# amazon-science/siam-mot

Measured on AMD Instinct MI355X. Metric: frame-pairs/sec at 720p, 30 active tracks; EMM xcorr HBM GB/s vs peak, higher is better.
Workload: dtype f32 (towers and correlation: fp16x2 operands on MFMA, fp32 accumulate, fp32-equivalent error); 1 GPU; EMM tracker-head frame pair (EMM.forward + EMM.extract_cache) on DLA-34-FPN 720p FPN maps (net input 704x1280, C=128, 5 levels), 30 tracks, one stream per GPU; hot path only: backbone / RPN / box head / solver are outside the timed region; tracks=30, channels=128, rz=15, rx=30, feature_sets=8, feature_bytes_rotated=307281920

## Files before the change

siam-mot_amd/csrc/sr_xcorr.hip:

```cpp
#include "pool_launch.h"
#include "xcorr_patch2.h"
#include "xcorr_patch1.h"
#include "xcorr_f16x2.h"
#include "knobs.h"
#include <type_traits>

namespace smot {

constexpr int FX_CH = 8;

struct SrOut {
    float* sr;
    float pad, half_e, two_e, min_wh;
    long long* trace;
    int abl;
    const int* n_valid;
    int order;
    float* hint_out;
    const float* hint_in;
    int hint_extra;
    int plan_pad[SMOT_MAX_LEVELS];
    float* plane_max;
};
constexpr int HINT_FLOATS = SMOT_HINT_FLOATS;
constexpr int HINT_BOUNDS = 8, HINT_GEOM = 12, HINT_YTAB = 16, HINT_XTAB = 16 + 256;
constexpr int HINT_BYROI = HINT_XTAB + 256, HINT_STATUS = HINT_BYROI + 6;
static_assert(HINT_BYROI + 8 == HINT_FLOATS && (HINT_FLOATS * 4) % 32 == 0 && HINT_STATUS == SMOT_HINT_STATUS_WORD,
              "hint entry layout");

typedef const __attribute__((address_space(1))) char* gptr_t;
__device__ __forceinline__ float ld_off(gptr_t base, unsigned byte_off) {
    return *reinterpret_cast<const __attribute__((address_space(1))) float*>(base + byte_off);
}
__device__ __forceinline__ gptr_t uniform_base(const float* p) {
    unsigned long long a = reinterpret_cast<unsigned long long>(p);
    asm volatile("" : "+s"(a));
    return reinterpret_cast<gptr_t>(a);
}

#ifdef SMOT_DEBUG
#include "../../measure/csrc/sr_xcorr_gen2.inc"
#endif

typedef int v4i_t __attribute__((ext_vector_type(4)));

typedef int v2i_t __attribute__((ext_vector_type(2)));
template <typename FT>
struct fx_pair {
    typedef int type;
};
template <>
struct fx_pair<float> {
    typedef v2i_t type;
};
template <typename FT>
__device__ __forceinline__ typename fx_pair<FT>::type fx_load2(__amdgpu_buffer_rsrc_t rsrc, unsigned voff, int soff) {
    if constexpr (sizeof(FT) == 4) {
        return __builtin_amdgcn_raw_buffer_load_b64(rsrc, voff, soff, 0);
    } else {
        return __builtin_amdgcn_raw_buffer_load_b32(rsrc, voff, soff, 0);
    }
}
template <typename FT>
__device__ __forceinline__ float fx_pair_elem(typename fx_pair<FT>::type v, int k) {
    if constexpr (sizeof(FT) == 4) {
        return __int_as_float(v[k]);
    } else {
        return k == 0 ? feat_of_pair<FT, 0>((unsigned)v) : feat_of_pair<FT, 1>((unsigned)v);
    }
}
template <typename FT>
__device__ __forceinline__ float fx_load1(__amdgpu_buffer_rsrc_t rsrc, unsigned voff, int soff) {
    if constexpr (sizeof(FT) == 4) {
        return __int_as_float(__builtin_amdgcn_raw_buffer_load_b32(rsrc, voff, soff, 0));
    } else {
        return feat_cvt<FT>((unsigned short)__builtin_amdgcn_raw_buffer_load_b16(rsrc, voff, soff, 0));
    }
}

__device__ __forceinline__ float rl_f(float v, int lane_const) {
    return __int_as_float(__builtin_amdgcn_readlane(__float_as_int(v), lane_const));
}

__device__ __forceinline__ float4 search_region_of(float b0, float b1, float b2, float b3, const SrOut& S) {
    const float bx1 = add_rn(b0, S.pad), by1 = add_rn(b1, S.pad);
    const float bx2 = add_rn(b2, S.pad), by2 = add_rn(b3, S.pad);
    const float bw = add_rn(sub_rn(bx2, bx1), 1.0f), bh = add_rn(sub_rn(by2, by1), 1.0f);
    const float w_ext = max_nan(div_rn(sub_rn(S.min_wh, bw), S.two_e), mul_rn(bw, S.half_e));
    const float h_ext = max_nan(div_rn(sub_rn(S.min_wh, bh), S.two_e), mul_rn(bh, S.half_e));
    return make_float4(sub_rn(bx1, w_ext), sub_rn(by1, h_ext), add_rn(bx2, w_ext), add_rn(by2, h_ext));
}

template <int RXN, int G>
__device__ __forceinline__ void fx_write_hint(const LevelParams& P, const float* __restrict__ boxes, const SrOut& S,
                                              const int* n_valid, float* hint_out, int NT, int x, int wave, int lane) {
    if (NT > 256 || wave >= 2) return;
    const int nv = (n_valid != nullptr) ? min(*n_valid + S.hint_extra, NT) : NT;
    if (x >= nv) return;
    unsigned long long mask[4][3];
    int cnt[3] = {0, 0, 0};
    int cl[4];
#pragma unroll
    for (int p = 0; p < 4; ++p) {
        const int t = lane + 64 * p;
        cl[p] = -1;
        if (64 * p < nv && t < nv) {
            const float4 b4 = *reinterpret_cast<const float4*>(boxes + (size_t)t * 4);
            int lvl = 0;
            if (P.num_levels > 1) lvl = map_level(boxes + (size_t)t * 4, P.k_min, P.k_max);
            float scale = P.scale[0];
#pragma unroll
            for (int l = 1; l < SMOT_MAX_LEVELS; ++l) scale = (lvl == l) ? P.scale[l] : scale;
            const float4 srb = search_region_of(b4.x, b4.y, b4.z, b4.w, S);
            const float ww = (srb.z - srb.x) * scale;
            cl[p] = ww <= 30.0f ? 0 : (ww <= 62.0f ? 1 : 2);
        }
#pragma unroll
        for (int c = 0; c < 3; ++c) {
            mask[p][c] = __ballot(cl[p] == c);
            cnt[c] += __popcll(mask[p][c]);
        }
    }
    const int px = x >> 6, lx = x & 63;
    int cx = 0;
#pragma unroll
    for (int p = 0; p < 4; ++p)
        if (p == px) cx = __builtin_amdgcn_readlane(cl[p], lx);
    int rank = cx == 2 ? 0 : (cx == 1 ? cnt[2] : cnt[2] + cnt[1]);
#pragma unroll
    for (int p = 0; p < 4; ++p) {
        const unsigned long long mk = cx == 2 ? mask[p][2] : (cx == 1 ? mask[p][1] : mask[p][0]);
        if (p < px) rank += __popcll(mk);
        if (p == px) rank += __popcll(mk & ((1ull << lx) - 1ull));
    }
    const float* bx = boxes + (size_t)x * 4;
    const float4 roi = search_region_of(bx[0], bx[1], bx[2], bx[3], S);
    int lvl = 0;
    if (P.num_levels > 1) lvl = map_level(bx, P.k_min, P.k_max);
    lvl = __builtin_amdgcn_readfirstlane(lvl);
    const int H = P.H[lvl], W = P.W[lvl], pad = S.plan_pad[lvl];
    const float scale = P.scale[lvl];
    const float x1 = mul_rn(roi.x, scale), y1 = mul_rn(roi.y, scale);
    const float x2 = mul_rn(roi.z, scale), y2 = mul_rn(roi.w, scale);
    const float bin_h = div_rn(fmaxf(sub_rn(y2, y1), 1.0f), (float)RXN);
    const float bin_w = div_rn(fmaxf(sub_rn(x2, x1), 1.0f), (float)RXN);
    int* ent = reinterpret_cast<int*>(hint_out) + (size_t)rank * HINT_FLOATS;
    int lo = 0, hi = 0;
    float wl = 0.0f, wh = 0.0f;
    if (lane < RXN * G) {
        if (wave == 0) {
            axis_sample(y1, bin_h, G, lane, H, pad, &lo, &hi, &wl, &wh);
        } else {
            axis_sample(x1, bin_w, G, lane, W, pad, &lo, &hi, &wl, &wh);
        }
    }
    int mn = 0x7fffffff, mx = -1;
    const unsigned long long m = __ballot(wl != 0.0f || wh != 0.0f);
    if (m != 0ull) {
        mn = __builtin_amdgcn_readlane((wl != 0.0f) ? lo : hi, __ffsll((long long)m) - 1);
        mx = __builtin_amdgcn_readlane((wh != 0.0f) ? hi : lo, 63 - __clzll((long long)m));
    }
    const int rl = (wl != 0.0f) ? lo : mn, rh = (wh != 0.0f) ? hi : mn;
    int4 e;
    if (wave == 0) {
        e.x = (int)((unsigned)(rl * W) * 4u);
        e.y = (int)((unsigned)(rh * W) * 4u);
    } else {
        e.x = (wl != 0.0f) ? lo - mn : 0;
        e.y = (wh != 0.0f) ? hi - mn : 0;
    }
    e.z = __float_as_int(wl);
    e.w = __float_as_int(wh);
    *reinterpret_cast<int4*>(ent + (wave == 0 ? HINT_YTAB : HINT_XTAB) + 4 * lane) = e;
    if (lane == 0) {
        ent[HINT_BOUNDS + 2 * wave] = mn;
        ent[HINT_BOUNDS + 2 * wave + 1] = mx;
        if (wave == 0) {
            float4* o = reinterpret_cast<float4*>(ent);
            o[0] = roi;
            o[1] = make_float4(__int_as_float(lvl), __int_as_float(x), 0.f, 0.f);
            ent[HINT_GEOM + 0] = pad;
            ent[HINT_GEOM + 1] = H;
            ent[HINT_GEOM + 2] = W;
            ent[HINT_GEOM + 3] = __float_as_int(scale);
            int* rec = reinterpret_cast<int*>(hint_out) + (size_t)x * HINT_FLOATS + HINT_BYROI;
            float4* r4 = reinterpret_cast<float4*>(rec);
            r4[0] = roi;
            rec[4] = lvl;
            rec[5] = nv;
            rec[6] = 0;
            rec[7] = 0;
        }
    }
}

__device__ __forceinline__ void fx_verify_hint(const LevelParams& P, const float* __restrict__ sr,
                                               const float* __restrict__ boxes, const float* hint, int x, int NT, int lane) {
    const int* rec = reinterpret_cast<const int*>(hint) + (size_t)x * HINT_FLOATS + HINT_BYROI;
    int v = 0;
    if (lane < 4) {
        v = __float_as_int(sr[(size_t)x * 4 + lane]);
    } else if (lane < 8) {
        v = __float_as_int(boxes[(size_t)x * 4 + lane - 4]);
    } else if (lane < 14) {
        v = rec[lane - 8];
    }
    const int up = __shfl_up(v, 8);
    float b4[4];
#pragma unroll
    for (int i = 0; i < 4; ++i) b4[i] = __int_as_float(__builtin_amdgcn_readlane(v, 4 + i));
    int lvl = 0;
    if (P.num_levels > 1) lvl = map_level(b4, P.k_min, P.k_max);
    const bool bad = (lane >= 8 && lane < 12 && up != v) || (lane == 12 && v != lvl) || (lane == 13 && v != NT);
    if (__ballot(bad) != 0ull && lane == 0)
        atomicOr(reinterpret_cast<int*>(const_cast<float*>(hint)) + HINT_STATUS, 1);
}

__device__ __forceinline__ bool fx_assign(const LevelParams& P, const float* __restrict__ sr,
                                          const float* __restrict__ boxes, const int* __restrict__ n_valid, int order,
                                          int by, int ny, const float* __restrict__ hint, int NT, int lane, int* n_out,
                                          int* cg_out, float4* roi_out, int* lvl_out, int* k_out) {
    int n = blockIdx.x, cg = by;
    *n_out = n;
    *cg_out = cg;
    if (order == 0 || NT > 256 || NT < 2) return false;
    const int T = NT * ny, L = by * NT + blockIdx.x;
    if (hint != nullptr && order == 1 && n_valid == nullptr) {
        const int k = L / ny;
        *cg_out = L - k * ny;
        *k_out = k;
        typedef int v8i_t __attribute__((ext_vector_type(8)));
        const v8i_t e = *reinterpret_cast<const __attribute__((address_space(4))) v8i_t*>(
            reinterpret_cast<unsigned long long>(hint) + (unsigned long long)k * (HINT_FLOATS * 4));
        roi_out->x = __int_as_float(e[0]);
        roi_out->y = __int_as_float(e[1]);
        roi_out->z = __int_as_float(e[2]);
        roi_out->w = __int_as_float(e[3]);
        *lvl_out = min(max(e[4], 0), P.num_levels - 1);
        *n_out = min(max(e[5], 0), NT - 1);
        return true;
    }
    const int nv = (n_valid != nullptr) ? min(*n_valid, NT) : NT;
    constexpr int SLOTS = 256;
    int i = L;
    if (order == 2) {
        const int r = L / SLOTS, q = L - r * SLOTS;
        if (r == 1) {
            i = T - 1 - q;
        } else if (r >= 2) {
            i = SLOTS + (L - 2 * SLOTS);
        }
    }
    int k;
    if (order == 3) {
        k = blockIdx.x;
    } else {
        k = i / ny;
        cg = i - k * ny;
    }
    *cg_out = cg;
    if (k >= nv) {
        *n_out = k;
        return false;
    }
    unsigned long long mask[4][3];
    int cnt[3] = {0, 0, 0};
    float rbx[4], rby[4], rbz[4], rbw[4];
    int rl[4];
#pragma unroll
    for (int p = 0; p < 4; ++p) {
        int cls = -1;
        const int t = lane + 64 * p;
        rbx[p] = rby[p] = rbz[p] = rbw[p] = 0.0f;
        rl[p] = 0;
        if (64 * p < nv && t < nv) {
            int lvl = 0;
            if (P.num_levels > 1) lvl = map_level(boxes + (size_t)t * 4, P.k_min, P.k_max);
            float scale = P.scale[0];
#pragma unroll
            for (int l = 1; l < SMOT_MAX_LEVELS; ++l) scale = (lvl == l) ? P.scale[l] : scale;
            const float4 b4 = *reinterpret_cast<const float4*>(sr + (size_t)t * 4);
            rbx[p] = b4.x;
            rby[p] = b4.y;
            rbz[p] = b4.z;
            rbw[p] = b4.w;
            rl[p] = lvl;
            const float ww = (b4.z - b4.x) * scale;
            cls = ww <= 30.0f ? 0 : (ww <= 62.0f ? 1 : 2);
        }
#pragma unroll
        for (int c = 0; c < 3; ++c) {
            mask[p][c] = __ballot(cls == c);
            cnt[c] += __popcll(mask[p][c]);
        }
    }
    int m = k, csel = 2;
    if (m >= cnt[2]) {
        m -= cnt[2];
        csel = 1;
        if (m >= cnt[1]) {
            m -= cnt[1];
            csel = 0;
        }
    }
    int psel = 0;
    bool done = false;
    unsigned long long msel = 0ull;
#pragma unroll
    for (int p = 0; p < 4; ++p) {
        const unsigned long long mk = csel == 2 ? mask[p][2] : (csel == 1 ? mask[p][1] : mask[p][0]);
        const int pc = __popcll(mk);
        if (!done) {
            if (m < pc) {
                psel = p;
                msel = mk;
                done = true;
            } else {
                m -= pc;
            }
        }
    }
    const unsigned long long below = msel & ((1ull << lane) - 1ull);
    const bool hit = ((msel >> lane) & 1ull) != 0ull && __popcll(below) == m;
    const unsigned long long b = __ballot(hit);
    if (b == 0ull) return false;
    const int ln = __ffsll((long long)b) - 1;
    *n_out = ln + 64 * psel;
    float sx = rbx[0], sy = rby[0], sz = rbz[0], sw = rbw[0];
    int lsel = rl[0];
#pragma unroll
    for (int p = 1; p < 4; ++p)
        if (psel == p) {
            sx = rbx[p];
            sy = rby[p];
            sz = rbz[p];
            sw = rbw[p];
            lsel = rl[p];
        }
    roi_out->x = __int_as_float(__builtin_amdgcn_readlane(__float_as_int(sx), ln));
    roi_out->y = __int_as_float(__builtin_amdgcn_readlane(__float_as_int(sy), ln));
    roi_out->z = __int_as_float(__builtin_amdgcn_readlane(__float_as_int(sz), ln));
    roi_out->w = __int_as_float(__builtin_amdgcn_readlane(__float_as_int(sw), ln));
    *lvl_out = __builtin_amdgcn_readlane(lsel, ln);
    return true;
}


#define FX_LEAD_PARAMS                                                                                                  \
    float *hint, const int *n_valid, const float *__restrict__ sr, const float *__restrict__ boxes,                     \
        long long *__restrict__ trace, int order, int grid_nx, int grid_ny, int C
#define FX_TAIL_PARAMS                                                                                                  \
    const float *__restrict__ z, float *__restrict__ resp, float *__restrict__ x_debug, int32_t *__restrict__ levels_out, \
        LevelParams P, SrOut S
template <int RX, int RZ, int G, bool XCORR, int NCH = FX_CH, bool P2 = false, int MM = 0>
__global__ void __launch_bounds__(64 * NCH, (P2 || MM == 1) ? 4 : 6)
sr_xcorr_fused9_kernel(FX_LEAD_PARAMS, FX_TAIL_PARAMS) {
    constexpr bool BATCHED = false;
    constexpr NoImages I{};
    using FT = float;
    constexpr bool NHWC = false;
#include "sr_xcorr_fused9_body.h"
}

template <int RX, int RZ, int G, bool XCORR, int NCH = FX_CH, int MM = 0>
__global__ void __launch_bounds__(64 * NCH, MM == 1 ? 4 : 6)
sr_xcorr_fused9_batched_kernel(FX_LEAD_PARAMS, FX_TAIL_PARAMS, ImageRows I) {
    constexpr bool BATCHED = true;
    constexpr bool P2 = false;
    using FT = float;
    constexpr bool NHWC = false;
#include "sr_xcorr_fused9_body.h"
}

template <typename FT, int RX, int RZ, int G, bool XCORR, int MM = 0>
__global__ void __launch_bounds__(64 * FX_CH, MM == 1 ? 4 : 6)
sr_xcorr_fused9_half_kernel(FX_LEAD_PARAMS, FX_TAIL_PARAMS) {
    static_assert(sizeof(FT) == 2, "fp16 / bf16 maps");
    constexpr bool BATCHED = false;
    constexpr NoImages I{};
    constexpr int NCH = FX_CH;
    constexpr bool P2 = false;
    constexpr bool NHWC = false;
#include "sr_xcorr_fused9_body.h"
}
// ... 246 lines not shown
```

siam-mot_amd/csrc/sr_xcorr_fused9_body.h:

```cpp
    constexpr int HO = XCORR ? RX - RZ + 1 : 16;
    constexpr int NS = RX * G;
    constexpr int XS = P2 ? XP2_XS : (MM == 2 ? XL_XS : XP1_XS), XP = P2 ? XP2_XP : (MM == 2 ? 30 * XL_XS : 32 * XP1_XS), ZS = XP1_ZS,
                  ZP = MM == 1 ? XH_TZ_FLOATS : (MM == 2 ? XL_TZ_FLOATS : RZ * XP1_ZS);
    static_assert(MM == 0 || (XCORR && !P2 && RX == 30 && RZ == 15), "the matrix-pipe correlation is the 30 / 15 head's");
    static_assert(MM != 2 || ((XP * 4) % 128 == 0 && ((2 * XP + 2 * ZP) * 4) % 128 == 0), "lean layout: 128-byte aligned plane images");
    constexpr int RH = (RX + 1) / 2;
    static_assert((!XCORR || RX - RZ + 1 == 16) && RX <= 32 && G == 2 && RX * XS <= XP && 2 * RH * G <= 64,
                  "specialised for pooled sizes <= 32, g = 2 (and the 30/15/16 correlation geometry)");
    __shared__ __attribute__((aligned(128))) float sm[(NCH / 2) * (2 * XP + 2 * ZP)];
    __shared__ __attribute__((aligned(16))) int4 tab[2][64 + 2 * RH * G];
    __shared__ int wbound[4];

    const int tid = threadIdx.x;
    const int lane = tid & 63;
    const int wave = __builtin_amdgcn_readfirstlane(tid >> 6);
    const float* const hint_in = XCORR ? hint : nullptr;
    float* const hint_out = XCORR ? nullptr : hint;
    const long long t_start = trace ? (long long)__builtin_amdgcn_s_memtime() : 0ll;
    float roi_early[4] = {0.0f, 0.0f, 0.0f, 0.0f};
    if constexpr (RX <= 15) {
#pragma unroll
        for (int k = 0; k < 4; ++k) roi_early[k] = sr[(size_t)blockIdx.x * 4 + k];
    }
    const int ka_h = P.H[0], ka_w = P.W[0], ka_p = P.pad[0];
    const float ka_s = P.scale[0];
    const unsigned long long ka_f = reinterpret_cast<unsigned long long>(P.feat[0]);
#define SMOT_KA_USE() asm volatile("" ::"s"(ka_h), "s"(ka_w), "s"(ka_p), "s"(ka_s), "s"(ka_f))
    int ka_i[6] = {0, 0, 0, 0, 0, 0};
    if constexpr (BATCHED) {
        ka_i[0] = I.num_images;
#pragma unroll
        for (int k = 1; k < 6; ++k) ka_i[k] = I.row_start[min(16 * k - 1, SMOT_MAX_IMAGES)];
    }
#ifdef SMOT_DEBUG
    if (S.abl >= 100 && (int)(blockIdx.y * grid_nx + blockIdx.x) >= 256) {
        for (int d = 0; d < S.abl - 100; ++d) __builtin_amdgcn_s_sleep(8);
    }
#endif
    int n_assigned, cg_assigned, lvl_assigned = 0;
    float4 roi_assigned = make_float4(0.f, 0.f, 0.f, 0.f);
    int grid_row = blockIdx.y, grid_rows = grid_ny;
    if constexpr (!XCORR) {
        if (hint_out != nullptr) {
            if (grid_row == 0) {
                fx_write_hint<30, G>(P, boxes, S, n_valid, hint_out, grid_nx, blockIdx.x, wave, lane);
                return;
            }
            grid_row -= 1;
            grid_rows -= 1;
        }
    }
    int4 tab_early = make_int4(0, 0, 0, 0);
    int4 ye_early = make_int4(0, 0, 0, 0), xe_early[2] = {make_int4(0, 0, 0, 0), make_int4(0, 0, 0, 0)};
    typedef int v8h_t __attribute__((ext_vector_type(8)));
    v8h_t g8 = {0, 0, 0, 0, -1, -1, -1, 0};
    if constexpr (XCORR && RX == 30) {
        if (hint_in != nullptr && order == 1 && n_valid == nullptr && grid_nx >= 2 && grid_nx <= 256) {
            const int k0 = (int)(blockIdx.y * grid_nx + blockIdx.x) / grid_ny;
            const int* ent = reinterpret_cast<const int*>(hint_in) + (size_t)k0 * HINT_FLOATS;
            g8 = *reinterpret_cast<const __attribute__((address_space(4))) v8h_t*>(
                reinterpret_cast<unsigned long long>(ent) + 4ull * HINT_BOUNDS);
            if (wave < 2) tab_early = *reinterpret_cast<const int4*>(ent + (wave == 0 ? HINT_YTAB : HINT_XTAB) + 4 * lane);
            if constexpr (MM == 1) {
                ye_early = *reinterpret_cast<const int4*>(ent + HINT_YTAB + 4 * min(lane + (wave & 1) * RH * G, 63));
                const int pwl = (lane & 31) < RX ? (lane & 31) : 0;
                xe_early[0] = *reinterpret_cast<const int4*>(ent + HINT_XTAB + 4 * (pwl * G));
                xe_early[1] = *reinterpret_cast<const int4*>(ent + HINT_XTAB + 4 * (pwl * G + 1));
            }
        }
    }
    if constexpr (XCORR && RX == 30) {
        if (hint_in != nullptr && order == 1 && n_valid == nullptr && grid_nx >= 2 && grid_nx <= 256 &&
            blockIdx.y == 0 && wave == 2
#ifdef SMOT_DEBUG
            && S.abl != 6
#endif
        )
            fx_verify_hint(P, sr, boxes, hint_in, blockIdx.x, grid_nx, lane);
    }
    int k_assigned = -1;
    const bool have_roi = fx_assign(P, sr, boxes, n_valid, RX > 15 ? order : 0, grid_row, grid_rows,
                                    XCORR ? hint_in : nullptr, grid_nx, lane, &n_assigned, &cg_assigned, &roi_assigned,
                                    &lvl_assigned, &k_assigned);
    SMOT_KA_USE();
#undef SMOT_KA_USE
    if constexpr (BATCHED)
        asm volatile("" ::"s"(ka_i[0]), "s"(ka_i[1]), "s"(ka_i[2]), "s"(ka_i[3]), "s"(ka_i[4]), "s"(ka_i[5]));
    const int n = __builtin_amdgcn_readfirstlane(n_assigned);
    const int cgrp = __builtin_amdgcn_readfirstlane(cg_assigned);
    if (n_valid != nullptr && n >= *n_valid) return;
    int img = 0;
    if constexpr (BATCHED) img = image_of_row(I, n);
#define FX_TRACE(SLOT)                                                                      \
    if (trace && tid == 0)                                                                  \
        trace[((size_t)n * grid_rows + cgrp) * 8 + (SLOT)] = (long long)__builtin_amdgcn_s_memtime();
    if (trace && tid == 0) trace[((size_t)n * grid_rows + cgrp) * 8 + 0] = t_start;
    FX_TRACE(5)

    float roi0 = roi_assigned.x, roi1 = roi_assigned.y, roi2 = roi_assigned.z, roi3 = roi_assigned.w;
    int lvl = lvl_assigned;
    if (!have_roi) {
        if constexpr (RX <= 15) {
            roi0 = roi_early[0];
            roi1 = roi_early[1];
            roi2 = roi_early[2];
            roi3 = roi_early[3];
        } else {
            roi0 = sr[(size_t)n * 4 + 0];
            roi1 = sr[(size_t)n * 4 + 1];
            roi2 = sr[(size_t)n * 4 + 2];
            roi3 = sr[(size_t)n * 4 + 3];
        }
        lvl = 0;
        if (P.num_levels > 1) lvl = map_level(boxes + (size_t)n * 4, P.k_min, P.k_max);
    }
    const float roi[4] = {roi0, roi1, roi2, roi3};
    lvl = __builtin_amdgcn_readfirstlane(lvl);
    if (levels_out != nullptr && cgrp == 0 && tid == 0) levels_out[n] = lvl;
    if (!XCORR && S.sr != nullptr && cgrp == 0 && tid == 0) {
        const float4 o = search_region_of(roi[0], roi[1], roi[2], roi[3], S);
        S.sr[n * 4 + 0] = o.x;
        S.sr[n * 4 + 1] = o.y;
        S.sr[n * 4 + 2] = o.z;
        S.sr[n * 4 + 3] = o.w;
    }
    const int H = P.H[lvl], W = P.W[lvl], pad = P.pad[lvl];
    const float scale = P.scale[lvl];
    const float x1 = mul_rn(roi[0], scale), y1 = mul_rn(roi[1], scale);
    const float x2 = mul_rn(roi[2], scale), y2 = mul_rn(roi[3], scale);
    const float bin_h = div_rn(fmaxf(sub_rn(y2, y1), 1.0f), (float)RX);
    const float bin_w = div_rn(fmaxf(sub_rn(x2, x1), 1.0f), (float)RX);
    FX_TRACE(6)
    constexpr int nplanes = NCH;
    const int c0 = cgrp * NCH;
    const bool owns = (wave < nplanes && c0 + wave < C);
    const int plane = n * C + c0 + wave;
    constexpr int NZ = XCORR ? (RZ * RZ + 63) / 64 : 1;
    float zreg[NZ];
    float zq[4] = {0.0f, 0.0f, 0.0f, 0.0f}, isz = 1.0f;
    if constexpr (MM != 0) {
        if (owns) xh_template_load(z + (size_t)plane * (RZ * RZ), lane, zq);
    } else if (XCORR && owns) {
        const float* __restrict__ zg = z + (size_t)plane * (RZ * RZ);
#pragma unroll
        for (int t = 0; t < NZ; ++t) zreg[t] = zg[min(lane + 64 * t, RZ * RZ - 1)];
    }

    const bool hent = XCORR && RX == 30 && k_assigned >= 0 && g8[4] == pad && g8[5] == H && g8[6] == W &&
                      g8[7] == __float_as_int(scale);
    const int hb[4] = {g8[0], g8[1], g8[2], g8[3]};
    const bool fast = !NHWC && MM == 1 && hent && hb[3] - hb[2] + 1 <= 64
#ifdef SMOT_DEBUG
                      && S.abl != 3 && S.abl != 12
#endif
        ;
    if (fast) {
    } else if (wave < 2 && hent) {
        tab[wave][lane] = tab_early;
        if (lane < 2 * RH * G) tab[wave][64 + lane] = make_int4(0, 0, 0, 0);
    } else if (wave < 2) {
        int lo = 0, hi = 0;
        float wl = 0.0f, wh = 0.0f;
        if (lane < NS) {
            if (wave == 0) {
                axis_sample(y1, bin_h, G, lane, H, pad, &lo, &hi, &wl, &wh);
            } else {
                axis_sample(x1, bin_w, G, lane, W, pad, &lo, &hi, &wl, &wh);
            }
        }
        int mn = 0x7fffffff, mx = -1;
        const unsigned long long m = __ballot(wl != 0.0f || wh != 0.0f);
        if (m != 0ull) {
            mn = __builtin_amdgcn_readlane((wl != 0.0f) ? lo : hi, __ffsll((long long)m) - 1);
            mx = __builtin_amdgcn_readlane((wh != 0.0f) ? hi : lo, 63 - __clzll((long long)m));
        }
        const int rl = (wl != 0.0f) ? lo : mn, rh = (wh != 0.0f) ? hi : mn;
        int4 e;
        if (wave == 0) {
            e.x = (int)((unsigned)(rl * W) * 4u);
            e.y = (int)((unsigned)(rh * W) * 4u);
        } else {
            e.x = (wl != 0.0f) ? lo - mn : 0;
            e.y = (wh != 0.0f) ? hi - mn : 0;
        }
        e.z = __float_as_int(wl);
        e.w = __float_as_int(wh);
        tab[wave][lane] = e;
        if (lane < 2 * RH * G) tab[wave][64 + lane] = make_int4(0, 0, 0, 0);
        if (lane == 0) {
            wbound[2 * wave] = mn;
            wbound[2 * wave + 1] = mx;
        }
    }
    FX_TRACE(7)
    if (!fast) __syncthreads();
    const int ymin = hent ? hb[0] : wbound[0], ymax = hent ? hb[1] : wbound[1];
    const int xmin = hent ? hb[2] : wbound[2], xmax = hent ? hb[3] : wbound[3];
    if (ymax < ymin || xmax < xmin) {
        if (owns) {
            if (XCORR) {
                for (int e = lane; e < HO * HO; e += 64) resp[(size_t)plane * HO * HO + e] = 0.0f;
                if (S.plane_max != nullptr && lane == 0) S.plane_max[plane] = 0.0f;
            }
            if (x_debug != nullptr)
                for (int e = lane; e < RX * RX; e += 64) x_debug[(size_t)plane * RX * RX + e] = 0.0f;
        }
        return;
    }
    const int ww = xmax - xmin + 1;
    FX_TRACE(1)

    if constexpr (MM != 0) {
    } else if (XCORR && owns) {
        float* zs = sm + (wave >> 1) * (2 * XP + 2 * ZP) + 2 * XP + (wave & 1) * ZP;
#pragma unroll
        for (int t = 0; t < NZ; ++t) {
            const int e = lane + 64 * t;
            if (e < RZ * RZ) {
                const int u = e / RZ;
                zs[u * ZS + (e - u * RZ)] = zreg[t];
            }
        }
    }
    FX_TRACE(2)

    const FT* __restrict__ fbase = reinterpret_cast<const FT*>(P.feat[lvl]);
    if constexpr (BATCHED) fbase += (size_t)img * ((size_t)C * H * W);
    const unsigned plane_bytes = (unsigned)(H * W) * (unsigned)sizeof(FT);
    constexpr int ROW_SHIFT = sizeof(FT) == 2 ? 1 : 0;
    auto pool = [&](auto pair_tag, auto chunk_tag, auto x2_tag, auto rows_tag) {
        constexpr bool PAIR = decltype(pair_tag)::value;
        constexpr bool CHUNKED = decltype(chunk_tag)::value;
        constexpr bool X2 = decltype(x2_tag)::value;
        constexpr int ROWS = decltype(rows_tag)::value;
        constexpr int NV = X2 ? 2 : 1;
        static_assert(!X2 || (PAIR && !CHUNKED), "two columns per lane is a form of the plane-pair mode");
        const int half = PAIR ? (lane >> 5) : 0;
        const int col = PAIR ? (lane & 31) : lane;
        const int pw = col < RX ? col : 0;
        const int pl0 = PAIR ? 2 * (wave >> 1) : wave;
        const bool has0 = (c0 + pl0 < C);
        const bool has1 = PAIR && (c0 + pl0 + 1 < C);
        if (!has0) return;
        const bool mine = PAIR ? (half == 0 || has1) : true;
        const unsigned lane_plane = (PAIR && half == 1 && has1) ? plane_bytes : 0u;
        float* xdst = sm + ((pl0 + half) >> 1) * (2 * XP + 2 * ZP) + ((pl0 + half) & 1) * XP;
        const FT* pbase = fbase + (size_t)(c0 + pl0) * H * W;
        unsigned long long pa = reinterpret_cast<unsigned long long>(pbase);
        const unsigned pa_lo = __builtin_amdgcn_readfirstlane((unsigned)pa);
        const unsigned pa_hi = __builtin_amdgcn_readfirstlane((unsigned)(pa >> 32));
        const auto rsrc = __builtin_amdgcn_make_buffer_rsrc(
            reinterpret_cast<void*>(((unsigned long long)pa_hi << 32) | pa_lo), 0, 0x7fffffff, 0x00020000);
        int sxl[G], sxh[G];
        float hxw[G], lxw[G];
#pragma unroll
        for (int ix = 0; ix < G; ++ix) {
            const int4 e = fast ? xe_early[ix] : tab[1][pw * G + ix];
            sxl[ix] = e.x;
            sxh[ix] = e.y;
            hxw[ix] = __int_as_float(e.z);
            lxw[ix] = __int_as_float(e.w);
        }
        const int row0 = PAIR ? (wave & 1) * RH : 0;
        const int nrows = PAIR ? RH : RX;
        const int nchunk = CHUNKED ? (ww + 63) >> 6 : 1;
        if constexpr (X2 && MM == 1) {
            constexpr int GR = (ROWS + 1) / 2, SW = 64;
            static_assert(RH % ROWS == 0 && GR * SW <= ROWS * XS, "full batches; staging fits a batch's own rows");
            const int wcol = min(2 * col, ww - 2);
            const unsigned voff = (unsigned)(xmin + wcol) * (unsigned)sizeof(FT) + lane_plane;
            typename fx_pair<FT>::type vl[ROWS][G], vh[ROWS][G];
            int4 ye = fast ? ye_early : tab[0][min(lane + row0 * G, 63 + 2 * RH * G)];
            ye.x = (int)((unsigned)ye.x >> ROW_SHIFT);
            ye.y = (int)((unsigned)ye.y >> ROW_SHIFT);
            int yoff = 0;
#define SMOT_FX_ISSUE()                                                                                             \
            _Pragma("unroll") for (int b = 0; b < ROWS; ++b)                                                        \
                _Pragma("unroll") for (int iy = 0; iy < G; ++iy) {                                                  \
                    vl[b][iy] = fx_load2<FT>(rsrc, voff, __builtin_amdgcn_readlane(ye.x, yoff + b * G + iy));         \
                    vh[b][iy] = fx_load2<FT>(rsrc, voff, __builtin_amdgcn_readlane(ye.y, yoff + b * G + iy));         \
                }
            SMOT_FX_ISSUE()
            __builtin_amdgcn_sched_barrier(0);
            if (owns) {
                unsigned char* tzw = reinterpret_cast<unsigned char*>(sm + (wave >> 1) * (2 * XP + 2 * ZP) + 2 * XP + (wave & 1) * ZP);
                isz = xh_template_store(zq, tzw, lane);
            }
            __builtin_amdgcn_sched_barrier(0);
#pragma unroll 1
            for (int r0 = row0; r0 < row0 + nrows; r0 += ROWS) {
                const float wl = __int_as_float(ye.z), wh = __int_as_float(ye.w);
                float cs[ROWS][NV];
#pragma unroll
                for (int b = 0; b < ROWS; ++b)
#pragma unroll
                    for (int k = 0; k < NV; ++k) {
                        float c_ = 0.0f;
#pragma unroll
                        for (int iy = 0; iy < G; ++iy) {
                            const int e = yoff + b * G + iy;
                            c_ = fmaf(rl_f(wl, e), fx_pair_elem<FT>(vl[b][iy], k), c_);
                            c_ = fmaf(rl_f(wh, e), fx_pair_elem<FT>(vh[b][iy], k), c_);
                        }
                        cs[b][k] = c_;
                    }
                __builtin_amdgcn_sched_barrier(0);
                if (r0 + ROWS < row0 + nrows) {
                    if (fast) yoff += ROWS * G;
                    else {
                        ye = tab[0][min(lane + (r0 + ROWS) * G, 63 + 2 * RH * G)];
                        ye.x = (int)((unsigned)ye.x >> ROW_SHIFT);
                        ye.y = (int)((unsigned)ye.y >> ROW_SHIFT);
                    }
                    SMOT_FX_ISSUE()
                }
                __builtin_amdgcn_sched_barrier(0);
                float acc[ROWS];
                float* stage = xdst + r0 * XS;
#pragma unroll
                for (int g0 = 0; g0 < ROWS; g0 += GR) {
#pragma unroll
                    for (int b = g0; b < g0 + GR && b < ROWS; ++b)
#pragma unroll
                        for (int k = 0; k < NV; ++k) stage[(b - g0) * SW + wcol + k] = cs[b][k];
                    float p[GR][G][2];
#pragma unroll
                    for (int b = g0; b < g0 + GR && b < ROWS; ++b)
#pragma unroll
                        for (int ix = 0; ix < G; ++ix) {
                            p[b - g0][ix][0] = stage[(b - g0) * SW + sxl[ix]];
                            p[b - g0][ix][1] = stage[(b - g0) * SW + sxh[ix]];
                        }
                    __builtin_amdgcn_sched_barrier(0);
#pragma unroll
                    for (int b = g0; b < g0 + GR && b < ROWS; ++b)
#pragma unroll
                        for (int ix = 0; ix < G; ++ix) {
                            acc[b] = fmaf(hxw[ix], p[b - g0][ix][0], ix == 0 ? 0.0f : acc[b]);
                            acc[b] = fmaf(lxw[ix], p[b - g0][ix][1], acc[b]);
                        }
                    __builtin_amdgcn_sched_barrier(0);
                }
#pragma unroll
                for (int b = 0; b < ROWS; ++b) {
                    const int ph = r0 + b;
                    if (col < RX && ph < row0 + nrows && ph < RX && mine) xdst[ph * XS + col] = acc[b] * (1.0f / (float)(G * G));
                }
            }
#undef SMOT_FX_ISSUE
            return;
        }
#pragma unroll 1
        for (int r0 = row0; r0 < row0 + nrows; r0 += ROWS) {
            const int4 ye = (fast && PAIR && !CHUNKED) ? ye_early : tab[0][min(lane + r0 * G, 63 + 2 * RH * G)];
            const unsigned ol = (unsigned)ye.x >> ROW_SHIFT, oh = (unsigned)ye.y >> ROW_SHIFT;
            const float wl = __int_as_float(ye.z), wh = __int_as_float(ye.w);
            float acc[ROWS];
            if (CHUNKED) {
#pragma unroll
                for (int b = 0; b < ROWS; ++b) acc[b] = 0.0f;
            }
#pragma unroll 1
            for (int ch = 0; ch < nchunk; ++ch) {
                const int cbase = ch << 6;
                const int wcol = CHUNKED ? min(cbase + col, ww - 1) : (X2 ? min(2 * col, ww - 2) : min(col, ww - 1));
                const unsigned voff = (unsigned)(xmin + wcol) * (unsigned)sizeof(FT) + lane_plane;
                float v[ROWS][G][2][NV];
#pragma unroll
                for (int b = 0; b < ROWS; ++b)
#pragma unroll
                    for (int iy = 0; iy < G; ++iy) {
                        const int e = b * G + iy;
                        if constexpr (X2) {
                            const auto l2 = fx_load2<FT>(rsrc, voff, __builtin_amdgcn_readlane((int)ol, e));
                            const auto h2 = fx_load2<FT>(rsrc, voff, __builtin_amdgcn_readlane((int)oh, e));
                            v[b][iy][0][0] = fx_pair_elem<FT>(l2, 0);
                            v[b][iy][0][NV - 1] = fx_pair_elem<FT>(l2, 1);
                            v[b][iy][1][0] = fx_pair_elem<FT>(h2, 0);
                            v[b][iy][1][NV - 1] = fx_pair_elem<FT>(h2, 1);
                        } else {
                            v[b][iy][0][0] = fx_load1<FT>(rsrc, voff, __builtin_amdgcn_readlane((int)ol, e));
                            v[b][iy][1][0] = fx_load1<FT>(rsrc, voff, __builtin_amdgcn_readlane((int)oh, e));
                        }
                    }
                __builtin_amdgcn_sched_barrier(0);
                if constexpr (MM != 0) {
                    if (r0 == row0 && ch == 0 && owns) {
                        unsigned char* tzw = reinterpret_cast<unsigned char*>(sm + (wave >> 1) * (2 * XP + 2 * ZP) + 2 * XP + (wave & 1) * ZP);
                        isz = MM == 2 ? xl_template_store(zq, tzw, lane) : xh_template_store(zq, tzw, lane);
                    }
                    __builtin_amdgcn_sched_barrier(0);
                }
                float cs[ROWS][NV];
#pragma unroll
                for (int b = 0; b < ROWS; ++b)
#pragma unroll
                    for (int k = 0; k < NV; ++k) {
                        float c_ = 0.0f;
#pragma unroll
                        for (int iy = 0; iy < G; ++iy) {
                            const int e = b * G + iy;
                            c_ = fmaf(rl_f(wl, e), v[b][iy][0][k], c_);
                            c_ = fmaf(rl_f(wh, e), v[b][iy][1][k], c_);
                        }
                        cs[b][k] = c_;
                    }
                __builtin_amdgcn_sched_barrier(0);
                constexpr int GR = ((P2 || MM == 2) && X2) ? 3 : (ROWS + 1) / 2;
                if constexpr (!CHUNKED) {
                    constexpr int SW = (X2 || !PAIR) ? 64 : 32;
                    static_assert(GR * SW <= (RH - (RH / ROWS) * ROWS == 0 ? ROWS : RH - (RH / ROWS) * ROWS) * XS,
                                  "staging fits the image rows of the wave's LAST batch");
                    float* stage = xdst + r0 * XS;
#pragma unroll
                    for (int g0 = 0; g0 < ROWS; g0 += GR) {
#pragma unroll
                        for (int b = g0; b < g0 + GR && b < ROWS; ++b)
#pragma unroll
                            for (int k = 0; k < NV; ++k) stage[(b - g0) * SW + wcol + k] = cs[b][k];
                        float p[GR][G][2];
#pragma unroll
                        for (int b = g0; b < g0 + GR && b < ROWS; ++b)
#pragma unroll
                            for (int ix = 0; ix < G; ++ix) {
                                p[b - g0][ix][0] = stage[(b - g0) * SW + sxl[ix]];
                                p[b - g0][ix][1] = stage[(b - g0) * SW + sxh[ix]];
                            }
                        __builtin_amdgcn_sched_barrier(0);
#pragma unroll
                        for (int b = g0; b < g0 + GR && b < ROWS; ++b)
#pragma unroll
                            for (int ix = 0; ix < G; ++ix) {
                                acc[b] = fmaf(hxw[ix], p[b - g0][ix][0], ix == 0 ? 0.0f : acc[b]);
                                acc[b] = fmaf(lxw[ix], p[b - g0][ix][1], acc[b]);
                            }
                        __builtin_amdgcn_sched_barrier(0);
                    }
                } else {
                    int al[G], ah[G];
                    bool inl[G], inh[G];
#pragma unroll
                    for (int ix = 0; ix < G; ++ix) {
                        const int tl = sxl[ix] - cbase, th = sxh[ix] - cbase;
                        inl[ix] = (unsigned)tl < 64u;
                        inh[ix] = (unsigned)th < 64u;
                        al[ix] = (tl & 63) << 2;
                        ah[ix] = (th & 63) << 2;
                    }
#pragma unroll
                    for (int g0 = 0; g0 < ROWS; g0 += GR) {
                        float p[GR][G][2];
#pragma unroll
                        for (int b = g0; b < g0 + GR && b < ROWS; ++b)
#pragma unroll
                            for (int ix = 0; ix < G; ++ix) {
                                p[b - g0][ix][0] = __int_as_float(__builtin_amdgcn_ds_bpermute(al[ix], __float_as_int(cs[b][0])));
                                p[b - g0][ix][1] = __int_as_float(__builtin_amdgcn_ds_bpermute(ah[ix], __float_as_int(cs[b][0])));
                            }
                        __builtin_amdgcn_sched_barrier(0);
#pragma unroll
                        for (int b = g0; b < g0 + GR && b < ROWS; ++b)
#pragma unroll
                            for (int ix = 0; ix < G; ++ix) {
                                acc[b] = inl[ix] ? fmaf(hxw[ix], p[b - g0][ix][0], acc[b]) : acc[b];
                                acc[b] = inh[ix] ? fmaf(lxw[ix], p[b - g0][ix][1], acc[b]) : acc[b];
                            }
                    }
                }
            }
#pragma unroll
            for (int b = 0; b < ROWS; ++b) {
                const int ph = r0 + b;
                if (col < RX && ph < row0 + nrows && ph < RX && mine) xdst[ph * XS + col] = acc[b] * (1.0f / (float)(G * G));
            }
        }
    };
    if constexpr (NHWC) {
#include "sr_pool_nhwc_stage.h"
    } else
    if (ww <= 32) {
        pool(std::true_type{}, std::false_type{}, std::false_type{}, std::integral_constant<int, RH>{});
#ifdef SMOT_DEBUG
    } else if (ww <= 64 && S.abl == 3 && MM != 2) {
        if constexpr (MM != 2) pool(std::false_type{}, std::false_type{}, std::false_type{}, std::integral_constant<int, RH>{});
#endif
    } else if (ww <= 64) {
        if constexpr (MM == 1) pool(std::true_type{}, std::false_type{}, std::true_type{}, std::integral_constant<int, RH / 3>{});
        else pool(std::true_type{}, std::false_type{}, std::true_type{}, std::integral_constant<int, (RH + 1) / 2>{});
    } else {
        pool(std::false_type{}, std::true_type{}, std::false_type{}, std::integral_constant<int, (RH + 2) / 3>{});
    }
    FX_TRACE(3)
    __syncthreads();
    if (x_debug != nullptr && owns) {
        const float* xs = sm + (wave >> 1) * (2 * XP + 2 * ZP) + (wave & 1) * XP;
        for (int e = lane; e < RX * RX; e += 64) {
            const int r = e / RX;
            x_debug[(size_t)plane * RX * RX + e] = xs[r * XS + (e - r * RX)];
        }
    }
    if constexpr (XCORR) {
#ifdef SMOT_DEBUG
        if (S.abl == 2) return;
#endif
        if constexpr (P2) {
            if (wave < nplanes / 2 && c0 + 2 * wave < C) {
                const float* xs2 = sm + wave * (2 * XP + 2 * ZP);
                xcorr_patch2_compute<RX, RZ, 0>(xs2, xs2 + 2 * XP, lane, resp, n * C + c0 + 2 * wave, n * C + min(C, c0 + NCH));
            }
        } else if (owns) {
            float* xs1 = sm + (wave >> 1) * (2 * XP + 2 * ZP) + (wave & 1) * XP;
            const float* zs1 = sm + (wave >> 1) * (2 * XP + 2 * ZP) + 2 * XP + (wave & 1) * ZP;
            if constexpr (MM == 1) xh_correlate<RX, RZ>(xs1, reinterpret_cast<const unsigned char*>(zs1), isz, lane, resp, plane, S.plane_max);
            else if constexpr (MM == 2) xl_correlate<RX, RZ>(xs1, reinterpret_cast<const unsigned char*>(zs1), isz, lane, resp, plane, S.plane_max);
            else xcorr_patch1_compute<RX, RZ, true>(xs1, zs1, lane, resp, plane, S.plane_max);
        }
    }
    FX_TRACE(4)
#undef FX_TRACE
```

Measured before the change: 18990 frame-pairs/s.

## Load contiguous row runs once and index them via GPR-indexed FMAs in pooling

Adds a fast path to the two-column plane-pair pooling. When a batch's vertical bilinear sample rows all fall inside a short contiguous run of feature rows, each row of the run is loaded once into a 32-register tuple. Per-sample rows are then picked with s_set_gpr_idx_on inline assembly and scalar weights, instead of issuing one buffer load per sample row pair. This is meant to remove duplicate global loads, since neighbouring samples share source rows. The cost is a ballot check, hand-written asm pinned to v32-v63 (register pressure), and a wave-uniform run-base assumption. The horizontal-tap code is moved into a shared lambda.

```diff
diff --git a/siam-mot_amd/csrc/sr_xcorr.hip b/siam-mot_amd/csrc/sr_xcorr.hip
--- a/siam-mot_amd/csrc/sr_xcorr.hip
+++ b/siam-mot_amd/csrc/sr_xcorr.hip
@@ -80,6 +80,54 @@
 
 __device__ __forceinline__ float rl_f(float v, int lane_const) {
     return __int_as_float(__builtin_amdgcn_readlane(__float_as_int(v), lane_const));
+}
+
+typedef float fx_rows_t __attribute__((ext_vector_type(32)));
+
+__device__ __forceinline__ void fx_run_fma4x2(const fx_rows_t r, int i0, int i1, int i2, int i3, float w0, float w1, float w2, float w3,
+                                              float* c0, float* c1) {
+    float a, b;
+    asm volatile("s_set_gpr_idx_on %3, gpr_idx(SRC0)\n\t"
+                 "v_fma_f32 %0, v32, %7, 0\n\t"
+                 "v_fma_f32 %1, v33, %7, 0\n\t"
+                 "s_set_gpr_idx_on %4, gpr_idx(SRC0)\n\t"
+                 "v_fma_f32 %0, v32, %8, %0\n\t"
+                 "v_fma_f32 %1, v33, %8, %1\n\t"
+                 "s_set_gpr_idx_on %5, gpr_idx(SRC0)\n\t"
+                 "v_fma_f32 %0, v32, %9, %0\n\t"
+                 "v_fma_f32 %1, v33, %9, %1\n\t"
+                 "s_set_gpr_idx_on %6, gpr_idx(SRC0)\n\t"
+                 "v_fma_f32 %0, v32, %10, %0\n\t"
+                 "v_fma_f32 %1, v33, %10, %1\n\t"
+                 "s_set_gpr_idx_off"
+                 : "=&v"(a), "=&v"(b)
+                 : "{v[32:63]}"(r), "s"(i0), "s"(i1), "s"(i2), "s"(i3), "s"(w0), "s"(w1), "s"(w2), "s"(w3));
+    *c0 = a;
+    *c1 = b;
+}
+
+template <int NE, int NB>
+__device__ __forceinline__ int fx_run_base(const int4 ye, const int lane) {
+    int base = __builtin_amdgcn_readlane(ye.x, 0);
+#pragma unroll
+    for (int b = 1; b < NB; ++b) base = lane >= b * NE ? __builtin_amdgcn_readlane(ye.x, b * NE) : base;
+    return base;
+}
+template <int NE, int NB>
+__device__ __forceinline__ bool fx_run_within(const int rows, const int4 ye, const int lane, const int n_real, const unsigned row_bytes) {
+    static_assert(NE * NB <= 64, "one lane per sample");
+    const int base = fx_run_base<NE, NB>(ye, lane);
+    const unsigned dl = (unsigned)(ye.x - base), dh = (unsigned)(ye.y - base), far = (unsigned)(rows - 1) * row_bytes;
+    const float wl = __int_as_float(ye.z), wh = __int_as_float(ye.w);
+    const bool ok = (dl <= far) & (dh <= far) & (wl == wl) & (wh == wh);
+    return row_bytes <= (1u << 18) && n_real > 0 && __ballot((lane < n_real) & !ok) == 0ull;
+}
+template <int NE, int NB, int NV>
+__device__ __forceinline__ void fx_run_index(const int4 ye, const int lane, const int n_real, const unsigned row_bytes, int* il, int* ih) {
+    const int base = fx_run_base<NE, NB>(ye, lane);
+    const float inv = __builtin_amdgcn_rcpf((float)row_bytes);
+    *il = lane < n_real ? NV * (int)((float)(unsigned)(ye.x - base) * inv + 0.5f) : 0;
+    *ih = lane < n_real ? NV * (int)((float)(unsigned)(ye.y - base) * inv + 0.5f) : 0;
 }
 
 __device__ __forceinline__ float4 search_region_of(float b0, float b1, float b2, float b3, const SrOut& S) {
diff --git a/siam-mot_amd/csrc/sr_xcorr_fused9_body.h b/siam-mot_amd/csrc/sr_xcorr_fused9_body.h
--- a/siam-mot_amd/csrc/sr_xcorr_fused9_body.h
+++ b/siam-mot_amd/csrc/sr_xcorr_fused9_body.h
@@ -228,6 +228,7 @@
     if constexpr (BATCHED) fbase += (size_t)img * ((size_t)C * H * W);
     const unsigned plane_bytes = (unsigned)(H * W) * (unsigned)sizeof(FT);
     constexpr int ROW_SHIFT = sizeof(FT) == 2 ? 1 : 0;
+    const unsigned row_bytes = (unsigned)W * 4u, last_row = (unsigned)(ymax * W) * 4u;
     auto pool = [&](auto pair_tag, auto chunk_tag, auto x2_tag, auto rows_tag) {
         constexpr bool PAIR = decltype(pair_tag)::value;
         constexpr bool CHUNKED = decltype(chunk_tag)::value;
@@ -271,10 +272,87 @@
             const unsigned voff = (unsigned)(xmin + wcol) * (unsigned)sizeof(FT) + lane_plane;
             typename fx_pair<FT>::type vl[ROWS][G], vh[ROWS][G];
             int4 ye = fast ? ye_early : tab[0][min(lane + row0 * G, 63 + 2 * RH * G)];
+            int yoff = 0;
+            auto htaps = [&](const float (&cs)[ROWS][NV], const int r0) {
+                float acc[ROWS];
+                float* stage = xdst + r0 * XS;
+#pragma unroll
+                for (int g0 = 0; g0 < ROWS; g0 += GR) {
+#pragma unroll
+                    for (int b = g0; b < g0 + GR && b < ROWS; ++b)
+#pragma unroll
+                        for (int k = 0; k < NV; ++k) stage[(b - g0) * SW + wcol + k] = cs[b][k];
+                    float p[GR][G][2];
+#pragma unroll
+                    for (int b = g0; b < g0 + GR && b < ROWS; ++b)
+#pragma unroll
+                        for (int ix = 0; ix < G; ++ix) {
+                            p[b - g0][ix][0] = stage[(b - g0) * SW + sxl[ix]];
+                            p[b - g0][ix][1] = stage[(b - g0) * SW + sxh[ix]];
+                        }
+                    __builtin_amdgcn_sched_barrier(0);
+#pragma unroll
+                    for (int b = g0; b < g0 + GR && b < ROWS; ++b)
+#pragma unroll
+                        for (int ix = 0; ix < G; ++ix) {
+                            acc[b] = fmaf(hxw[ix], p[b - g0][ix][0], ix == 0 ? 0.0f : acc[b]);
+                            acc[b] = fmaf(lxw[ix], p[b - g0][ix][1], acc[b]);
+                        }
+                    __builtin_amdgcn_sched_barrier(0);
+                }
+#pragma unroll
+                for (int b = 0; b < ROWS; ++b) {
+                    const int ph = r0 + b;
+                    if (col < RX && ph < row0 + nrows && ph < RX && mine) xdst[ph * XS + col] = acc[b] * (1.0f / (float)(G * G));
+                }
+            };
+            constexpr int NE = ROWS * G, RMAX = NE + 2;
+            static_assert(RMAX * NV <= 32, "a run fits the register tuple");
+            if (fx_run_within<NE, RH / ROWS>(RMAX, ye, lane, RH * G, row_bytes)) {
+                int il, ih;
+                fx_run_index<NE, RH / ROWS, NV>(ye, lane, RH * G, row_bytes, &il, &ih);
+                fx_rows_t rr;
+#define SMOT_FX_ISSUE_RUN()                                                                                         \
+                {                                                                                                   \
+                    const unsigned rb_ = (unsigned)__builtin_amdgcn_readlane(ye.x, yoff);                           \
+                    _Pragma("unroll") for (int j = 0; j < RMAX; ++j) {                                              \
+                        const auto v2_ = fx_load2<FT>(rsrc, voff, (int)(min(rb_ + j * row_bytes, last_row) >> ROW_SHIFT)); \
+                        rr[NV * j] = fx_pair_elem<FT>(v2_, 0);                                                      \
+                        rr[NV * j + 1] = fx_pair_elem<FT>(v2_, 1);                                                  \
+                    }                                                                                               \
+                }
+                SMOT_FX_ISSUE_RUN()
+                __builtin_amdgcn_sched_barrier(0);
+                if (owns) {
+                    unsigned char* tzw = reinterpret_cast<unsigned char*>(sm + (wave >> 1) * (2 * XP + 2 * ZP) + 2 * XP + (wave & 1) * ZP);
+                    isz = xh_template_store(zq, tzw, lane);
+                }
+                __builtin_amdgcn_sched_barrier(0);
+#pragma unroll 1
+                for (int r0 = row0; r0 < row0 + nrows; r0 += ROWS) {
+                    const float wl = __int_as_float(ye.z), wh = __int_as_float(ye.w);
+                    float cs[ROWS][NV];
+#pragma unroll
+                    for (int b = 0; b < ROWS; ++b) {
+                        const int e = yoff + b * G;
+                        const int i0 = __builtin_amdgcn_readlane(il, e), i1 = __builtin_amdgcn_readlane(ih, e);
+                        const int i2 = __builtin_amdgcn_readlane(il, e + 1), i3 = __builtin_amdgcn_readlane(ih, e + 1);
+                        fx_run_fma4x2(rr, i0, i1, i2, i3, rl_f(wl, e), rl_f(wh, e), rl_f(wl, e + 1), rl_f(wh, e + 1), &cs[b][0], &cs[b][1]);
+                    }
+                    __builtin_amdgcn_sched_barrier(0);
+                    if (r0 + ROWS < row0 + nrows) {
+                        yoff += NE;
+                        SMOT_FX_ISSUE_RUN()
+                    }
+                    __builtin_amdgcn_sched_barrier(0);
+                    htaps(cs, r0);
+                }
+#undef SMOT_FX_ISSUE_RUN
+                return;
+            }
             ye.x = (int)((unsigned)ye.x >> ROW_SHIFT);
             ye.y = (int)((unsigned)ye.y >> ROW_SHIFT);
-            int yoff = 0;
-#define SMOT_FX_ISSUE()                                                                                             \
+#define SMOT_FX_ISSUE()                                                                                           \
             _Pragma("unroll") for (int b = 0; b < ROWS; ++b)                                                        \
                 _Pragma("unroll") for (int iy = 0; iy < G; ++iy) {                                                  \
                     vl[b][iy] = fx_load2<FT>(rsrc, voff, __builtin_amdgcn_readlane(ye.x, yoff + b * G + iy));         \
@@ -315,37 +393,7 @@
                     SMOT_FX_ISSUE()
                 }
                 __builtin_amdgcn_sched_barrier(0);
-                float acc[ROWS];
-                float* stage = xdst + r0 * XS;
-#pragma unroll
-                for (int g0 = 0; g0 < ROWS; g0 += GR) {
-#pragma unroll
-                    for (int b = g0; b < g0 + GR && b < ROWS; ++b)
-#pragma unroll
-                        for (int k = 0; k < NV; ++k) stage[(b - g0) * SW + wcol + k] = cs[b][k];
-                    float p[GR][G][2];
-#pragma unroll
-                    for (int b = g0; b < g0 + GR && b < ROWS; ++b)
-#pragma unroll
-                        for (int ix = 0; ix < G; ++ix) {
-                            p[b - g0][ix][0] = stage[(b - g0) * SW + sxl[ix]];
-                            p[b - g0][ix][1] = stage[(b - g0) * SW + sxh[ix]];
-                        }
-                    __builtin_amdgcn_sched_barrier(0);
-#pragma unroll
-                    for (int b = g0; b < g0 + GR && b < ROWS; ++b)
-#pragma unroll
-                        for (int ix = 0; ix < G; ++ix) {
-                            acc[b] = fmaf(hxw[ix], p[b - g0][ix][0], ix == 0 ? 0.0f : acc[b]);
-                            acc[b] = fmaf(lxw[ix], p[b - g0][ix][1], acc[b]);
-                        }
-                    __builtin_amdgcn_sched_barrier(0);
-                }
-#pragma unroll
-                for (int b = 0; b < ROWS; ++b) {
-                    const int ph = r0 + b;
-                    if (col < RX && ph < row0 + nrows && ph < RX && mine) xdst[ph * XS + col] = acc[b] * (1.0f / (float)(G * G));
-                }
+                htaps(cs, r0);
             }
 #undef SMOT_FX_ISSUE
             return;
```

Result: faster. 19420 frame-pairs/s, median of 6 (+2.3%).
